# alexoz12v2/cuda-optix-pathtracing

Measured on AMD Instinct MI355X. Metric: Msamples/s (paths x spp / s), higher is better.
Workload: dtype f32

## Files before the change

### cuda-optix-pathtracing_amd/binding.py

```python
import ctypes as C
import subprocess
from pathlib import Path

import numpy as np

_HERE = Path(__file__).resolve().parent
_CSRC = _HERE / "csrc"
_LIB = None

DMT_ACCEL_BRUTE_FORCE = 0
DMT_ACCEL_BVH = 1
BVH_BUILD_HOST = 0
BVH_BUILD_DEVICE = 1
BVH_BUILT_BY_HOST = 0
BVH_BUILT_BY_DEVICE = 1
BVH_BUILT_BY_HOST_AFTER_DEVICE = 2
BVH_UPDATE_REBUILD = 0
BVH_UPDATE_REFIT = 1
BVH_UPDATE_AUTO = 2
BVH_UPDATED_NONE = 0
BVH_UPDATED_REFIT = 1
BVH_UPDATED_REBUILD = 2
BVH_UPDATED_REBUILD_AFTER_REFIT = 3


class DmtError(RuntimeError):
    pass


def library_path():
    import os
    alt = os.environ.get("DMT_HIP_LIB")
    return Path(alt) if alt else _CSRC / "libdmt_hip.so"


def build_library(force=False):
    args = ["make", "-C", str(_CSRC)]
    if force:
        args.append("-B")
    subprocess.check_call(args)
    return library_path()


def load_library():
    global _LIB
    if _LIB is None:
        so = library_path()
        if not so.exists():
            raise DmtError(f"{so} is missing: run `python -c 'import __graft_entry__ as g; g.build()'` "
                           "(the HIP path has no fallback)")
        lib = C.CDLL(str(so))
        lib.dmt_last_error.restype = C.c_char_p
        lib.dmt_last_error.argtypes = [C.c_void_p]
        _LIB = lib
    return _LIB


EXPORTED_SYMBOLS = [
    "dmt_ctx_create", "dmt_ctx_destroy", "dmt_last_error", "dmt_upload_triangles", "dmt_upload_bsdfs",
    "dmt_upload_lights", "dmt_set_camera", "dmt_set_limits", "dmt_set_accel", "dmt_set_light_sampling", "dmt_light_tree_pmfs", "dmt_light_tree_ref_select", "dmt_set_bvh_strategy", "dmt_set_partition", "dmt_set_chunk", "dmt_render_profile",
    "dmt_upload_area_lights", "dmt_upload_textures", "dmt_upload_envmap", "dmt_clear_envmap", "dmt_envmap_tables", "dmt_test_envmap",
    "dmt_set_stream", "dmt_film_clear", "dmt_film_bind", "dmt_film_device_ptrs", "dmt_download_film",
    "dmt_render", "dmt_render_adaptive", "dmt_render_stats", "dmt_sync", "dmt_sched_diag", "dmt_kernel_time", "dmt_kernel_info", "dmt_bvh_validate", "dmt_brute_cull_plan", "dmt_brute_cull_box_plan", "dmt_test_triangle_intersect",
    "dmt_test_sampler", "dmt_test_camera_rays", "dmt_test_bsdf", "dmt_test_bsdf_ng", "dmt_test_material", "dmt_test_light", "dmt_test_half",
    "dmt_test_trace_samples", "dmt_test_trace_log", "dmt_test_closest_hit",
    "dmt_set_texture_filter", "dmt_texture_mip_chain", "dmt_texture_footprint", "dmt_test_texture_filter",
    "dmt_render_aovs", "dmt_upload_aovs", "dmt_download_aovs", "dmt_denoise_defaults", "dmt_denoise",
    "dmt_set_accel_build", "dmt_accel_build_info", "dmt_accel_download", "dmt_lbvh_reference", "dmt_bvh_check",
    "dmt_update_vertices", "dmt_update_vertices_device", "dmt_set_accel_update", "dmt_accel_update_info", "dmt_bvh_refit_reference",
    "dmt_download_aov_surface", "dmt_upload_aov_surface", "dmt_camera_project", "dmt_test_camera_project", "dmt_temporal_defaults",
    "dmt_denoise_temporal", "dmt_temporal_reset", "dmt_temporal_info", "dmt_temporal_download",
    "dmt_set_sampler_table", "dmt_sampler_table_plan", "dmt_test_sampler_table",
]

SAMPLER_TABLE_OFF = 0
SAMPLER_TABLE_AUTO = 1
SAMPLER_TABLE_FORCE = 2


class SamplerTablePlanRecord(C.Structure):
    _fields_ = [("use", C.c_uint32), ("period_width", C.c_uint32), ("period_height", C.c_uint32), ("entry_bytes", C.c_uint32),
                ("slices", C.c_uint32), ("reserved", C.c_uint32), ("slice_bytes", C.c_uint64)]


def sampler_table_plan(width, height, owned_pixels, spp, chunk_spp, budget_bytes=0, mode=SAMPLER_TABLE_AUTO):
    lib = load_library()
    rec = SamplerTablePlanRecord()
    args = [int(width), int(height), C.c_uint64(int(owned_pixels)), C.c_uint32(int(spp)), C.c_uint32(int(chunk_spp)),
            C.c_uint64(int(budget_bytes)), int(mode)]
    rc = lib.dmt_sampler_table_plan(*args, C.byref(rec), None, C.c_uint32(0))
    if rc != 0:
        raise DmtError(f"dmt_sampler_table_plan failed ({rc})")
    lens = (C.c_uint32 * max(int(rec.slices), 1))()
    rc = lib.dmt_sampler_table_plan(*args, C.byref(rec), lens, C.c_uint32(int(rec.slices)))
    if rc != 0:
        raise DmtError(f"dmt_sampler_table_plan failed ({rc})")
    out = {name: int(getattr(rec, name)) for name, _ in SamplerTablePlanRecord._fields_ if name != "reserved"}
    out["use"] = bool(rec.use)
    out["slice_spp"] = [int(x) for x in lens[:int(rec.slices)]]
    return out


class DenoiseParams(C.Structure):
    _fields_ = [("iterations", C.c_int32), ("sigma_normal", C.c_float), ("sigma_position", C.c_float),
                ("sigma_albedo", C.c_float), ("sigma_luminance", C.c_float)]


def denoise_defaults():
    lib = load_library()
    lib.dmt_denoise_defaults.restype = DenoiseParams
    p = lib.dmt_denoise_defaults()
    return {name: getattr(p, name) for name, _ in DenoiseParams._fields_}



class TemporalParams(C.Structure):
    _fields_ = [("alpha", C.c_float), ("normal_threshold", C.c_float), ("plane_threshold", C.c_float)]


class TemporalRecord(C.Structure):
    _fields_ = [("frames", C.c_uint32), ("reprojected", C.c_uint32), ("reset", C.c_uint32), ("temporal_ms", C.c_float),
                ("history_bytes", C.c_uint64)]


def temporal_defaults():
    lib = load_library()
    lib.dmt_temporal_defaults.restype = TemporalParams
    p = lib.dmt_temporal_defaults()
    return {name: getattr(p, name) for name, _ in TemporalParams._fields_}


def camera_project(camera44, points):
    lib = load_library()
    cam = np.ascontiguousarray(camera44, np.uint8).reshape(44)
    p = np.ascontiguousarray(points, np.float32).reshape(-1, 3)
    xy, depth = np.zeros((p.shape[0], 2), np.float32), np.zeros(p.shape[0], np.float32)
    rc = lib.dmt_camera_project(cam.ctypes.data_as(C.c_void_p), int(p.shape[0]), p.ctypes.data_as(C.c_void_p),
                                xy.ctypes.data_as(C.c_void_p), depth.ctypes.data_as(C.c_void_p))
    if rc != 0:
        raise DmtError(f"dmt_camera_project failed ({rc})")
    return xy, depth


TEXFILTER_LEVEL0 = 0
TEXFILTER_REFERENCE = 1


def mip_level_count(width, height):
# ... 565 lines not shown
        prep = np.zeros((n, 12), np.float32)
        samp = np.zeros((n, 10), np.float32)
        ev = np.zeros((n, 4), np.float32)
        self._check(self._lib.dmt_test_bsdf_ng(self._ctx, _p(b), n, _p(ns), _p(ng), _p(wo), _p(u2), _p(uc), _p(wi_eval),
                                               _p(prep), _p(samp), _p(ev)), "dmt_test_bsdf_ng")
        return prep, samp, ev

    def test_material(self, tri, bu, bv, ng):
        tri, bu, bv, ng = _i32(tri), _f32(bu, (-1,)), _f32(bv, (-1,)), _f32(ng, (-1, 3))
        n = tri.shape[0]
        assert bu.shape[0] == n and bv.shape[0] == n and ng.shape[0] == n
        rec, rec2 = np.zeros((n, 32), np.uint8), np.zeros((n, 32), np.uint8)
        ns = np.zeros((n, 3), np.float32)
        mix = np.zeros(n, np.float32)
        self._check(self._lib.dmt_test_material(self._ctx, n, _p(tri), _p(bu), _p(bv), _p(ng), _p(rec), _p(ns), _p(rec2),
                                                _p(mix)), "dmt_test_material")
        return rec, ns, rec2, mix

    def test_light(self, light32, pos, nrm, u2, had_t):
        l = np.ascontiguousarray(light32, np.uint8).reshape(32)
        pos, nrm, u2 = _f32(pos, (-1, 3)), _f32(nrm, (-1, 3)), _f32(u2, (-1, 2))
        ht = _i32(had_t)
        n = pos.shape[0]
        out = np.zeros((n, 14), np.float32)
        self._check(self._lib.dmt_test_light(self._ctx, _p(l), n, _p(pos), _p(nrm), _p(u2), _p(ht), _p(out)),
                    "dmt_test_light")
        return out

    def test_half(self, floats=None, halves=None):
        h_out = f_out = None
        n = 0
        if floats is not None:
            floats = _f32(floats, (-1,))
            n = floats.shape[0]
            h_out = np.zeros(n, np.uint16)
        if halves is not None:
            halves = np.ascontiguousarray(halves, np.uint16).reshape(-1)
            n = halves.shape[0]
            f_out = np.zeros(n, np.float32)
        if floats is not None and halves is not None:
            assert floats.shape[0] == halves.shape[0]
        self._check(self._lib.dmt_test_half(self._ctx, n, _p(floats), _p(h_out), _p(halves), _p(f_out)),
                    "dmt_test_half")
        return h_out, f_out

    def test_trace_samples(self, pxs, pys, ss):
        pxs, pys, ss = _i32(pxs), _i32(pys), _i32(ss)
        n = pxs.shape[0]
        out = np.zeros((n, 3), np.float32)
        self._check(self._lib.dmt_test_trace_samples(self._ctx, n, _p(pxs), _p(pys), _p(ss), _p(out)),
                    "dmt_test_trace_samples")
        return out

    def test_texture_filter(self, tri, bu, bv, tex, depth=0):
        tri, tex = _i32(tri), _i32(tex)
        bu, bv = _f32(bu), _f32(bv)
        n = tri.shape[0]
        tex = np.ascontiguousarray(np.broadcast_to(tex, (n,)), np.int32)
        depth = np.ascontiguousarray(np.broadcast_to(_i32(depth), (n,)), np.int32)
        assert bu.shape[0] == n and bv.shape[0] == n
        rgb = np.zeros((n, 3), np.float32)
        branch = np.zeros(n, np.int32)
        lod = np.zeros(n, np.float32)
        self._check(self._lib.dmt_test_texture_filter(self._ctx, n, _p(tri), _p(bu), _p(bv), _p(tex), _p(depth), _p(rgb),
                                                      _p(branch), _p(lod)), "dmt_test_texture_filter")
        return rgb, branch, lod

    def test_trace_log(self, px, py, s, cap=64):
        rec = np.zeros((cap, 12), np.float32)
        n = C.c_int()
        L = np.zeros(3, np.float32)
        self._check(self._lib.dmt_test_trace_log(self._ctx, int(px), int(py), int(s), _p(rec), int(cap), C.byref(n),
                                                 _p(L)), "dmt_test_trace_log")
        return rec[:n.value], L

    def test_closest_hit(self, o, d):
        o, d = _f32(o, (-1, 3)), _f32(d, (-1, 3))
        n = o.shape[0]
        idx = np.zeros(n, np.int32)
        t = np.zeros(n, np.float32)
        self._check(self._lib.dmt_test_closest_hit(self._ctx, n, _p(o), _p(d), _p(idx), _p(t)),
                    "dmt_test_closest_hit")
        return idx, t
```

### cuda-optix-pathtracing_amd/csrc/dmt_hip.hip

```cpp
#include <hip/hip_runtime.h>

#include <algorithm>
#include <chrono>
#include <cmath>
#include <cstddef>
#include <cstdio>
#include <cstdlib>
#include <cstring>
#include <limits>
#include <memory>
#include <new>
#include <string>
#include <vector>

#include "../../include/dmt_hip.h"
#include "pt_device.hpp"
#include "bvh_device.hpp"
#include "bvh_gpu_build.hpp"
#include "devbuf.hpp"
#include "envmap.hpp"
#include "light_tree.hpp"
#include "light_tree_ref.hpp"

using namespace dmt;
// ... 835 lines not shown
        }
        set_shadow_ray(st, offset_ray_origin(hit.pos, hit.error, hit.normal, ls.direction), ls.direction);
        st.smax = ls.distance;
        st.hasShadow = true;
      }
    }
  }

  sect_mark(7);
  f2 const u2 = st.rng.get2D();
  float const uc = st.rng.get1D();
  BsdfSample bs = sample_bsdf(b, wo, ns, hit.normal, u2, uc);
  if constexpr (F & kFeatBlend) {
    if (blend) {
      BsdfSample sC = sample_bsdf(b2, wo, ns, hit.normal, u2, uc);
      sC.f = bs.f * (1.f - mix) + sC.f * mix;
      sC.pdf = blend_pdf(bs.pdf, sC.pdf);
      sC.eta = 1.f;
      bs = sC;
    }
  }
  sect_mark(8);
  if (!bs.valid()) return true;
  st.lastT = bs.refract;
  if constexpr (F & (kFeatEnv | kFeatArea)) st.lastPdf = bs.pdf, st.lastSpecular = bs.delta;
  set_ray(st, offset_ray_origin(hit.pos, hit.error, hit.normal, bs.wi), bs.wi);
  st.beta = st.beta * (bs.f * fabsf(dot(bs.wi, hit.normal)) / bs.pdf);
  float const rrBeta = max3(st.beta * bs.eta);
  if (rrBeta < 1 && st.depth > 1) {
    float const q = fmaxf(0.f, 1.f - rrBeta);
    if (st.rng.get1D() < q) return true;
    st.beta = st.beta / (1 - q);
  }
  ++st.depth;
  sect_mark(9);
  return false;
}

DMT_DEV TriS load_tri(TriIsect const DMT_CONST_AS* tris, uint32_t i) {
  TriS T;
  T.p0x = tris[i].p0x, T.p0y = tris[i].p0y, T.p0z = tris[i].p0z;
  T.e0x = tris[i].e0x, T.e0y = tris[i].e0y, T.e0z = tris[i].e0z;
  T.e1x = tris[i].e1x, T.e1y = tris[i].e1y, T.e1z = tris[i].e1z;
  return T;
}

struct BruteHit {
  float bt, bu, bv;
  int tri;
  bool occluded;
};
#define DMT_TRI_DECL(P) float P##0, P##1, P##2, P##3, P##4, P##5, P##6, P##7, P##8
#define DMT_TRI_LOAD(P, idx)                                                                          \
  P##0 = tris[idx].p0x, P##1 = tris[idx].p0y, P##2 = tris[idx].p0z, P##3 = tris[idx].e0x, P##4 = tris[idx].e0y, \
  P##5 = tris[idx].e0z, P##6 = tris[idx].e1x, P##7 = tris[idx].e1y, P##8 = tris[idx].e1z
#define DMT_TRI_TEST(P, idx)                                                                                   \
  do {                                                                                                         \
    MTPair m;                                                                                                  \
    mt_core9<v2f>(P##0, P##1, P##2, P##3, P##4, P##5, P##6, P##7, P##8, st.rp.ox, st.rp.oy, st.rp.oz, st.rp.dx, \
                  st.rp.dy, st.rp.dz, m.det, m.t, m.u, m.v);                                                   \
    bool const v1 = mt_valid(m.det.x, m.t.x, m.u.x, m.v.x);                                                    \
    bool const v2 = mt_valid(m.det.y, m.t.y, m.u.y, m.v.y);                                                    \
    if (doC && v1 && m.t.x < h.bt) {                  \
      h.bt = m.t.x;                                                                                            \
      h.tri = int(idx);                                                                                        \
      h.bu = m.u.x;                                                                                            \
      h.bv = m.v.x;                                                                                            \
    }                                                                                                          \
    if (doS && v2 && m.t.y < st.smax) h.occluded = true;                                         \
  } while (0)

__shared__ float s_cullTri[9 * kCullMaxTris];
__shared__ CullRec s_cullRec[kCullMaxClusters];
__shared__ unsigned long long s_cullKey[kLdsThreads];
__shared__ unsigned long long s_cullOcc[kLdsThreads / 64];
__shared__ uint8_t s_cullOwner[kLdsThreads / 64][kCullGroup][128];
constexpr float kCullTSlack = 1.0f + 1.0f / 256;
constexpr float kCullRel = 1.0f / 16384;
constexpr float kCullTLo = 1e-4f * (1.0f - 1.0f / 256);

#ifndef DMT_CULL_COUNTS
#define DMT_CULL_COUNTS 0
#endif
#if DMT_CULL_COUNTS
__device__ unsigned long long g_cullCount[16];
#endif

DMT_DEV void cull_stage(KArgs k) {
  k = kargs(k);
  if (k->cull.clusterCount == 0) return;
  float const* const t9 = k->cull.tri9;
  for (uint32_t i = threadIdx.x; i < 9 * kCullMaxTris; i += blockDim.x) s_cullTri[i] = t9[i];
  CullCluster const* const cl = k->cull.clusters;
  for (uint32_t i = threadIdx.x; i < kCullMaxClusters; i += blockDim.x)
    s_cullRec[i] = CullRec{cl[i].first, cl[i].count | cl[i].slot << 16, cl[i].magic};
  __syncthreads();
}

DMT_DEV float slab_rcp(float d) { return rcp_(copysignf(fmaxf(fabsf(d), 0x1p-126f), d)); }

DMT_DEV void brute_clusters(KArgs k, PathState const& st, bool doC, bool doS, BruteHit& h) {
  k = kargs(k);
  uint32_t const nc = k->cull.clusterCount;
  auto const* const cls = to_const_as(k->cull.clusters);
  if (h.tri >= 0) h.tri = int(k->cull.alwaysIdx[h.tri]);
  uint32_t const lane = threadIdx.x & 63u, w = threadIdx.x >> 6;
  unsigned long long const act = __ballot(1);
  uint32_t const nAct = uint32_t(__popcll(act));
  uint32_t const rank = __builtin_amdgcn_mbcnt_hi(uint32_t(act >> 32), __builtin_amdgcn_mbcnt_lo(uint32_t(act), 0u));
  s_cullKey[threadIdx.x] = ~0ull;
  s_cullOcc[w] = 0;
  float tmaxC = h.bt * kCullTSlack;
  float const tmaxS = st.smax * kCullTSlack;
  v2f const ix = {slab_rcp(st.rp.dx.x), slab_rcp(st.rp.dx.y)};
  v2f const iy = {slab_rcp(st.rp.dy.x), slab_rcp(st.rp.dy.y)};
  v2f const iz = {slab_rcp(st.rp.dz.x), slab_rcp(st.rp.dz.y)};
#if DMT_CULL_COUNTS
  unsigned long long cnt[16] = {};
  cnt[0] = 1, cnt[1] = __popcll(__ballot(doC)), cnt[2] = __popcll(__ballot(doS));
#endif
  for (uint32_t c0 = 0; c0 < nc; c0 += kCullGroup) {
    uint32_t pre[kCullGroup + 1];
    pre[0] = 0;
#pragma unroll
    for (uint32_t q = 0; q < kCullGroup; ++q) {
      uint32_t tasks = 0;
      if (c0 + q < nc) {
        auto const& r = cls[c0 + q];
        CullCluster cl;
        for (int i = 0; i < 6; ++i) cl.b[i] = r.b[i];
        cl.box = r.box, cl.count = r.count;
        bool hitC, hitS;
        if (cl.box) {
          v2f const x0 = (cl.b[0] - st.rp.ox) * ix, x1 = (cl.b[3] - st.rp.ox) * ix;
          v2f const y0 = (cl.b[1] - st.rp.oy) * iy, y1 = (cl.b[4] - st.rp.oy) * iy;
          v2f const z0 = (cl.b[2] - st.rp.oz) * iz, z1 = (cl.b[5] - st.rp.oz) * iz;
          float const nC = fmaxf(fmaxf(fminf(x0.x, x1.x), fminf(y0.x, y1.x)), fmaxf(fminf(z0.x, z1.x), kCullTLo));
          float const fC = fminf(fminf(fmaxf(x0.x, x1.x), fmaxf(y0.x, y1.x)), fminf(fmaxf(z0.x, z1.x), tmaxC));
          float const nS = fmaxf(fmaxf(fminf(x0.y, x1.y), fminf(y0.y, y1.y)), fmaxf(fminf(z0.y, z1.y), kCullTLo));
          float const fS = fminf(fminf(fmaxf(x0.y, x1.y), fmaxf(y0.y, y1.y)), fminf(fmaxf(z0.y, z1.y), tmaxS));
          hitC = doC && nC <= fC * kCullTSlack, hitS = doS && nS <= fS * kCullTSlack;
        } else {
          v2f const wx = cl.b[0] - st.rp.ox, wy = cl.b[1] - st.rp.oy, wz = cl.b[2] - st.rp.oz;
          v2f const dd = st.rp.dx * st.rp.dx + st.rp.dy * st.rp.dy + st.rp.dz * st.rp.dz;
          v2f const ww = wx * wx + wy * wy + wz * wz;
          v2f tc = (wx * st.rp.dx + wy * st.rp.dy + wz * st.rp.dz) * rcp_(dd);
          tc.x = fminf(fmaxf(tc.x, 0.f), tmaxC);
          tc.y = fminf(fmaxf(tc.y, 0.f), tmaxS);
          v2f const ex = wx - tc * st.rp.dx, ey = wy - tc * st.rp.dy, ez = wz - tc * st.rp.dz;
          v2f const ee = ex * ex + ey * ey + ez * ez;
          v2f const lim = cl.b[3] + kCullRel * (ww + tc * tc * dd);
          hitC = doC && ee.x <= lim.x, hitS = doS && ee.y <= lim.y;
        }
        unsigned long long const mC = __ballot(hitC), mS = __ballot(hitS);
        uint32_t const nC = uint32_t(__popcll(mC)), nS = uint32_t(__popcll(mS));
        if (hitC) s_cullOwner[w][q][__builtin_amdgcn_mbcnt_hi(uint32_t(mC >> 32), __builtin_amdgcn_mbcnt_lo(uint32_t(mC), 0u))] = uint8_t(lane);
        if (hitS)
          s_cullOwner[w][q][nC + __builtin_amdgcn_mbcnt_hi(uint32_t(mS >> 32), __builtin_amdgcn_mbcnt_lo(uint32_t(mS), 0u))] =
              uint8_t(lane | 64u);
        tasks = (nC + nS) * cl.count;
#if DMT_CULL_COUNTS
        if (cl.box) cnt[5] += nC, cnt[7] += nS, cnt[9] += tasks;
        else cnt[4] += nC, cnt[6] += nS, cnt[8] += tasks;
#endif
      }
      pre[q + 1] = pre[q] + tasks;
    }
    uint32_t const total = pre[kCullGroup];
#if DMT_CULL_COUNTS
    cnt[3] += (total + nAct - 1) / nAct;
#endif
    asm volatile("" ::: "memory");
    for (uint32_t base = 0; base < total; base += nAct) {
      uint32_t const g = min(base + rank, total - 1u);
      uint32_t q = 0, first = 0;
#pragma unroll
      for (uint32_t p = 1; p < kCullGroup; ++p)
        if (g >= pre[p]) q = p, first = pre[p];
      CullRec const rec = s_cullRec[c0 + q];
      uint32_t const count = rec.countSlot & 0xFFFFu, slot0 = rec.countSlot >> 16;
      uint32_t const local = g - first;
      uint32_t const e = __umulhi(local, rec.magic);
      uint32_t const j = local - e * count;
      uint32_t const own = s_cullOwner[w][q][e];
      bool const shadow = own >= 64u;
      int const src = int(own & 63u) << 2;
      auto pull = [&](v2f v) {
        float const a = __int_as_float(__builtin_amdgcn_ds_bpermute(src, __float_as_int(v.x)));
        float const b = __int_as_float(__builtin_amdgcn_ds_bpermute(src, __float_as_int(v.y)));
        return shadow ? b : a;
      };
      float const ox = pull(st.rp.ox), oy = pull(st.rp.oy), oz = pull(st.rp.oz);
      float const dx = pull(st.rp.dx), dy = pull(st.rp.dy), dz = pull(st.rp.dz);
      float const smax = __int_as_float(__builtin_amdgcn_ds_bpermute(src, __float_as_int(st.smax)));
      float const* const T = s_cullTri + slot0 + j;
      float det, t, u, v;
      mt_core9<float>(T[0 * kCullMaxTris], T[1 * kCullMaxTris], T[2 * kCullMaxTris], T[3 * kCullMaxTris], T[4 * kCullMaxTris],
                      T[5 * kCullMaxTris], T[6 * kCullMaxTris], T[7 * kCullMaxTris], T[8 * kCullMaxTris], ox, oy, oz, dx, dy, dz,
                      det, t, u, v);
      if (base + rank < total && mt_valid(det, t, u, v)) {
        if (shadow) {
          if (t < smax) atomicOr(&s_cullOcc[w], 1ull << (own & 63u));
        } else if (t < kInf) {
          atomicMin(&s_cullKey[w * 64u + own],
                    (static_cast<unsigned long long>(__float_as_uint(t)) << 32) | ((rec.first + j) << kCullSlotBits) | (slot0 + j));
        }
      }
    }
    asm volatile("" ::: "memory");
    if (c0 + kCullGroup < nc) {
      unsigned long long const kc = s_cullKey[threadIdx.x];
      if (kc != ~0ull) tmaxC = fminf(tmaxC, __uint_as_float(uint32_t(kc >> 32)) * kCullTSlack);
    }
  }
#if DMT_CULL_COUNTS
  if (rank == 0)
    for (int i = 0; i < 10; ++i) atomicAdd(&g_cullCount[i], cnt[i]);
#endif
  if (doC) {
    unsigned long long const kc = s_cullKey[threadIdx.x];
    if (kc < ((static_cast<unsigned long long>(__float_as_uint(h.bt)) << 32) | (uint32_t(h.tri) << kCullSlotBits))) {
      float const* const T = s_cullTri + (uint32_t(kc) & ((1u << kCullSlotBits) - 1u));
      float det, t, u, v;
      mt_core9<float>(T[0 * kCullMaxTris], T[1 * kCullMaxTris], T[2 * kCullMaxTris], T[3 * kCullMaxTris], T[4 * kCullMaxTris],
                      T[5 * kCullMaxTris], T[6 * kCullMaxTris], T[7 * kCullMaxTris], T[8 * kCullMaxTris], st.rp.ox.x, st.rp.oy.x,
                      st.rp.oz.x, st.rp.dx.x, st.rp.dy.x, st.rp.dz.x, det, t, u, v);
      h.bt = __uint_as_float(uint32_t(kc >> 32)), h.tri = int(uint32_t(kc) >> kCullSlotBits), h.bu = u, h.bv = v;
    }
  }
  if (doS && ((s_cullOcc[w] >> lane) & 1ull)) h.occluded = true;
}

template <bool CULL>
DMT_DEV void trace_pair_brute(KArgs k, PathState const& st, bool doC, bool doS, int& bestTri, float& bu,
                              float& bv, bool& occluded) {
  BruteHit h{kInf, 0.f, 0.f, -1, false};
  k = kargs(k);
  auto const* tris = to_const_as(CULL ? k->cull.always : k->scene.tris);
  uint32_t const n = CULL ? k->cull.alwaysCount : k->scene.triCount;
  uint32_t const last = n ? n - 1 : 0;
  DMT_TRI_DECL(a);
  DMT_TRI_DECL(b);
  DMT_TRI_LOAD(a, 0);
  for (uint32_t i = 0; i < n;) {
    uint32_t const ib = i + 1 < last ? i + 1 : last;
    DMT_TRI_LOAD(b, ib);
    __builtin_amdgcn_sched_barrier(0);
    DMT_TRI_TEST(a, i);
    if (++i >= n) break;
    uint32_t const ia = i + 1 < last ? i + 1 : last;
    DMT_TRI_LOAD(a, ia);
    __builtin_amdgcn_sched_barrier(0);
    DMT_TRI_TEST(b, i);
    ++i;
  }
  if constexpr (CULL) {
    if (kargs(k)->cull.clusterCount != 0) brute_clusters(k, st, doC, doS, h);
  }
  bestTri = h.tri, bu = h.bu, bv = h.bv, occluded = h.occluded;
}

struct LaneStats {
  uint32_t samples = 0, closest = 0, shadow = 0, bounces = 0;
  TraversalCounters tc;
  uint32_t itNode = 0, itLeaf = 0, itShade = 0, itOuter = 0, itPrep = 0, lanesLeaf = 0, lanesShade = 0, lanesPrep = 0;
};
template <bool STATS = false>
DMT_DEV void trace_pair_bvh(KArgs k, PathState const& st, bool doC, bool doS, uint32_t gtid, int& bestTri,
                            float& bu, float& bv, bool& occluded, LaneStats* ls = nullptr) {
  BvhView const bvh = load_bvh(k);
  float bt;
  if constexpr (STATS) ls->closest += doC ? 1u : 0u, ls->shadow += doS ? 1u : 0u;
  bvh_closest<STATS>(bvh, doC, mk3(st.rp.ox.x, st.rp.oy.x, st.rp.oz.x), mk3(st.rp.dx.x, st.rp.dy.x, st.rp.dz.x),
                     gtid, bestTri, bt, bu, bv, STATS ? &ls->tc : nullptr);
  occluded = bvh_any<STATS>(bvh, doS, mk3(st.rp.ox.y, st.rp.oy.y, st.rp.oz.y),
                            mk3(st.rp.dx.y, st.rp.dy.y, st.rp.dz.y), st.smax, gtid, STATS ? &ls->tc : nullptr);
}

template <uint32_t F, class Sink>
DMT_DEV void lane_finish(KArgs k, PathState& st, bool doC, bool doS, int bestTri, float bu, float bv, bool occluded,
                         Sink&& sink);

template <uint32_t F, class Sink>
DMT_DEV void lane_step(KArgs k, uint32_t gtid, PathState& st, Sink&& sink, LaneStats* ls = nullptr) {
  bool const doC = st.active;
  bool const doS = st.hasShadow;
  int bestTri;
  float bu, bv;
  bool occluded;
  if constexpr (F & kFeatBvh)
    trace_pair_bvh<(F & kFeatStats) != 0>(k, st, doC, doS, gtid, bestTri, bu, bv, occluded, ls);
  else
    trace_pair_brute(k, st, doC, doS, bestTri, bu, bv, occluded);
  sect_mark(2);
  if constexpr (F & kFeatStats) ls->bounces += (doC && bestTri >= 0 && st.depth < kargs(k)->maxDepth) ? 1u : 0u;
  lane_finish<F & ~kFeatStats>(k, st, doC, doS, bestTri, bu, bv, occluded, sink);
}

template <uint32_t F, class Sink>
DMT_DEV void lane_finish(KArgs k, PathState& st, bool doC, bool doS, int bestTri, float bu, float bv, bool occluded,
// ... 3204 lines not shown
```

### cuda-optix-pathtracing_amd/csrc/probes.hpp

```cpp
#pragma once

#include "probe_stage.hpp"

namespace {

template <uint32_t F>
__global__ void k_test_trace(RenderParams P, int n, int32_t const* pxs, int32_t const* pys, int32_t const* ss, float* L3) {
  KArgs const k = kargs_base();
  if constexpr (!(F & kFeatBvh)) cull_stage(k);
  int const i = int(blockIdx.x * blockDim.x + threadIdx.x);
  PathState st{};
  if (i < n) {
    ColdArgs const c = load_cold_args(k);
    path_begin(st, c.cam, c.sp, pxs[i], pys[i], halton_pixel_base(c.sp, pxs[i], pys[i]), uint32_t(ss[i]));
  }
  auto store = [&](f3 L, uint32_t) { L3[3 * i] = L.x, L3[3 * i + 1] = L.y, L3[3 * i + 2] = L.z; };
  uint32_t const gtid = blockIdx.x * blockDim.x + threadIdx.x;
  while (__any(st.active || st.hasShadow)) lane_step<F>(k, gtid, st, store);
}

__global__ void k_test_texfilter(RenderParams P, int n, int32_t const* tri, float const* bu, float const* bv, int32_t const* tex,
                                 int32_t const* depth, float* rgb3, int32_t* branch, float* lod) {
#pragma clang fp contract(off)
  KArgs const k = kargs_base();
// ... 149 lines not shown
__global__ void k_test_bsdf(Rec32 rec, int n, float const* ns3, float const* wo3, float const* u2, float const* uc, float const* wi3,
                            float* prep12, float* samp10, float* eval4) {
  test_bsdf_body<false>(rec, n, ns3, nullptr, wo3, u2, uc, wi3, prep12, samp10, eval4);
}

__global__ void k_test_bsdf_ng(Rec32 rec, int n, float const* ns3, float const* ng3, float const* wo3, float const* u2,
                               float const* uc, float const* wi3, float* prep12, float* samp10, float* eval4) {
  test_bsdf_body<true>(rec, n, ns3, ng3, wo3, u2, uc, wi3, prep12, samp10, eval4);
}

__global__ void k_test_material(RenderParams P, int n, int32_t const* tri, float const* bu, float const* bv, float const* ng3,
                                uint32_t* rec8, float* ns3, uint32_t* rec2_8, float* mixOut) {
  KArgs const k = kargs_base();
  int const i = int(blockIdx.x * blockDim.x + threadIdx.x);
  if (i >= n) return;
  SceneView const sc = load_scene(k);
  uint32_t const matId = sc.post[tri[i]].matId;
  f3 const ng = mk3(ng3[3 * i], ng3[3 * i + 1], ng3[3 * i + 2]);
  Rec32 rec = sc.bsdfs[matId], rec2{};
  float mix = 0.f;
  bool const blend = hi16(rec.w[1]) == BS_GGX_BLEND && matId + 1u < sc.bsdfCount;
  if (blend) {
    mix = blend_metallic<false>(k, rec, matId, tri[i], bu[i], bv[i]);
    rec.w[1] = (rec.w[1] & 0x0000FFFFu) | (uint32_t(BS_GGX_DIEL) << 16);
    rec2 = sc.bsdfs[matId + 1u];
  }
  f3 ns = ng;
  if (kargs(k)->matTex != nullptr) {
    ns = apply_material_textures<false>(k, rec, matId, tri[i], bu[i], bv[i], ng);
    if (blend) (void)apply_material_textures<false>(k, rec2, matId + 1u, tri[i], bu[i], bv[i], ng);
  }
  if (blend) rec.w[1] = (rec.w[1] & 0x0000FFFFu) | (uint32_t(BS_GGX_BLEND) << 16);
  for (int w = 0; w < 8; ++w) rec8[8 * size_t(i) + w] = rec.w[w], rec2_8[8 * size_t(i) + w] = rec2.w[w];
  ns3[3 * i] = ns.x, ns3[3 * i + 1] = ns.y, ns3[3 * i + 2] = ns.z;
  mixOut[i] = mix;
}

__global__ void k_test_light(Rec32 rec, int n, float const* pos3, float const* nrm3, float const* u2,
                             int32_t const* hadT, float* out14) {
  int const i = int(blockIdx.x * blockDim.x + threadIdx.x);
  if (i >= n) return;
  LightSample const s = sample_light(rec, mk3(pos3[3 * i], pos3[3 * i + 1], pos3[3 * i + 2]),
                                     mk2(u2[2 * i], u2[2 * i + 1]), hadT[i] != 0,
                                     mk3(nrm3[3 * i], nrm3[3 * i + 1], nrm3[3 * i + 2]));
  f3 const Le = eval_light(rec, s);
  float* o = out14 + 14 * size_t(i);
  o[0] = s.pLight.x, o[1] = s.pLight.y, o[2] = s.pLight.z;
  o[3] = s.direction.x, o[4] = s.direction.y, o[5] = s.direction.z;
  o[6] = s.pdf, o[7] = float(s.delta), o[8] = s.distance, o[9] = s.factor;
  o[10] = Le.x, o[11] = Le.y, o[12] = Le.z, o[13] = s.valid() ? 1.f : 0.f;
}

__global__ void k_test_half(int n, float const* fin, uint16_t* hout, uint16_t const* hin, float* fout) {
  int const i = int(blockIdx.x * blockDim.x + threadIdx.x);
  if (i >= n) return;
  if (fin && hout) hout[i] = uint16_t(f2h(fin[i]));
  if (hin && fout) fout[i] = h2f(hin[i]);
}

__global__ void k_test_closest(RenderParams P, bool useBvh, int n, float const* o3, float const* d3, int32_t* tri,
                               float* tOut) {
  KArgs const k = kargs_base();
  if (!useBvh) cull_stage(k);
  int const i = int(blockIdx.x * blockDim.x + threadIdx.x);
  bool const alive = i < n;
  PathState st{};
  if (alive)
    set_ray(st, mk3(o3[3 * i], o3[3 * i + 1], o3[3 * i + 2]), mk3(d3[3 * i], d3[3 * i + 1], d3[3 * i + 2]));
  st.active = alive;
  int best;
  float bu, bv, bt = kInf;
  bool occluded;
  if (useBvh)
    trace_pair_bvh(k, st, alive, false, blockIdx.x * blockDim.x + threadIdx.x, best, bu, bv, occluded);
  else
    trace_pair_brute(k, st, alive, false, best, bu, bv, occluded);
  if (alive && best >= 0) {
    TriS const T = load_tri(to_const_as(load_scene(k).tris), uint32_t(best));
    bt = mt_pair(T, st.rp).t.x;
  }
  if (alive) tri[i] = best, tOut[i] = bt;
}

__global__ void k_test_project(ProjXf c, int n, float const* p3, float* xy2, float* depth) {
  int const i = int(blockIdx.x * blockDim.x + threadIdx.x);
  if (i >= n) return;
  Proj const o = project_point(c, p3[3 * i], p3[3 * i + 1], p3[3 * i + 2]);
  xy2[2 * i] = o.fx, xy2[2 * i + 1] = o.fy, depth[i] = o.depth;
}

typedef void (*TestTraceFn)(RenderParams, int, int32_t const*, int32_t const*, int32_t const*, float*);
#define DMT_TEST_TRACE_ROW(suffix, mask, waves, body) {mask, k_test_trace<mask>},
KernelRow<TestTraceFn> const kTestTraceKernels[] = {DMT_MEGAKERNELS(DMT_TEST_TRACE_ROW)};

int probeError(dmt_ctx* ctx, Probe const& p) {
  ctx->err = std::string(p.call) + ": " + hipGetErrorName(p.err) + " - " + hipGetErrorString(p.err);
  return DMT_ERR_HIP;
}

int finishProbe(dmt_ctx* ctx, Probe& p) {
  if (int const rc = finishTest(ctx)) return rc;
  return p.fetch() == hipSuccess ? DMT_OK : probeError(ctx, p);
}

int sceneReady(dmt_ctx* ctx, char const* who, bool wholeScene) {
  if (wholeScene && !(ctx->haveTris && ctx->haveBsdfs && ctx->haveLights && ctx->haveCamera))
    return fail(ctx, DMT_ERR_STATE, (std::string(who) + ": scene/camera not set").c_str());
  if (ctx->triCount > 0 && ctx->maxMatId >= ctx->bsdfCount)
    return fail(ctx, DMT_ERR_INVALID, (std::string(who) + ": material index outside the BSDF array").c_str());
  return DMT_OK;
}

int probeBsdf(dmt_ctx* ctx, void const* bsdf32, int n, float const* ns3, float const* ng3, float const* wo3, float const* u2,
              float const* uc, float const* wi_eval3, float* prepared12, float* sample10, float* eval4) {
  if (n == 0) return DMT_OK;
  Probe p(ctx->device, size_t(n));
  ProbeIn<float> dns(p, ns3, 3), dng(p, ng3, 3), dwo(p, wo3, 3), du2(p, u2, 2), duc(p, uc, 1), dwi(p, wi_eval3, 3);
  ProbeOut<float> dp(p, prepared12, 12), ds(p, sample10, 10), de(p, eval4, 4);
  if (p.err != hipSuccess) return probeError(ctx, p);
  Rec32 rec;
  memcpy(&rec, bsdf32, 32);
  if (ng3)
    hipLaunchKernelGGL(k_test_bsdf_ng, dim3(p.blocks(64)), dim3(64), 0, ctx->stream, rec, n, dns.get(), dng.get(), dwo.get(), du2.get(),
                       duc.get(), dwi.get(), dp.get(), ds.get(), de.get());
  else
    hipLaunchKernelGGL(k_test_bsdf, dim3(p.blocks(64)), dim3(64), 0, ctx->stream, rec, n, dns.get(), dwo.get(), du2.get(), duc.get(),
                       dwi.get(), dp.get(), ds.get(), de.get());
  return finishProbe(ctx, p);
}

}

extern "C" {

int dmt_test_envmap(dmt_ctx* ctx, int n, const float* u2, const float* wi_in3, float* wi3, float* pdf, float* uv2, float* Le3,
                    int32_t* ok, float* Le_dir3, float* pdf_dir) {
  if (!ctx || n <= 0 || !u2 || !wi_in3 || !wi3 || !pdf || !uv2 || !Le3 || !ok || !Le_dir3 || !pdf_dir) return DMT_ERR_INVALID;
  if (ctx->env.w <= 0) return fail(ctx, DMT_ERR_STATE, "dmt_test_envmap: no env map uploaded");
  Probe p(ctx->device, size_t(n));
  ProbeIn<float> du(p, u2, 2), dwin(p, wi_in3, 3);
  ProbeOut<float> dwi(p, wi3, 3), dpdf(p, pdf, 1), duv(p, uv2, 2), dLe(p, Le3, 3), dLd(p, Le_dir3, 3), dpd(p, pdf_dir, 1);
  ProbeOut<int32_t> dok(p, ok, 1);
  if (p.err != hipSuccess) return probeError(ctx, p);
  hipLaunchKernelGGL(k_test_envmap, dim3(p.blocks(64)), dim3(64), 0, ctx->stream, ctx->env, n, du.get(), dwin.get(), dwi.get(),
                     dpdf.get(), duv.get(), dLe.get(), dok.get(), dLd.get(), dpd.get());
  return finishProbe(ctx, p);
}

int dmt_test_sampler_table(dmt_ctx* ctx, int width, int height, uint32_t s0, uint32_t n, float* out_vals, float* out_jitter) {
  if (!ctx || width <= 0 || height <= 0 || !out_vals || !out_jitter) return DMT_ERR_INVALID;
  uint32_t const pw = uint32_t(width < 128 ? width : 128), ph = uint32_t(height < 128 ? height : 128);
  SamplerParams const sp = computeSamplerParams(width, height);
  if (uint64_t(n) * pw * ph > 0x7FFFFFFFull || (uint64_t(s0) + n + 1) * uint64_t(sp.scale0) * uint64_t(sp.scale1) > 0x7FFFFFFFull)
    return fail(ctx, DMT_ERR_INVALID, "dmt_test_sampler_table: too many entries, or the sample index overflows the 32-bit Halton index");
  if (n == 0) return DMT_OK;
  Probe p(ctx->device, size_t(n) * pw * ph);
  ProbeOut<float4> dv(p, out_vals, 2);
  ProbeOut<float2> dj(p, out_jitter, 1);
  if (p.err != hipSuccess) return probeError(ctx, p);
  hipLaunchKernelGGL(k_sampler_table, dim3(p.blocks(256)), dim3(256), 0, ctx->stream, sp, s0, n, pw, ph, dv.get(), dj.get());
  return finishProbe(ctx, p);
}

int dmt_test_triangle_intersect(dmt_ctx* ctx, const float* xs, const float* ys, const float* zs, size_t count, const float* o3,
                                const float* d3, int32_t* hit, float* t, float* pos3, float* nrm3, float* err3) {
  if (!ctx || !xs || !ys || !zs || !o3 || !d3 || !hit) return DMT_ERR_INVALID;
// ... 104 lines not shown
  if (n == 0) return DMT_OK;
  Probe p(ctx->device, size_t(n));
  ProbeIn<float> dfi(p, f_in, 1);
  ProbeOut<uint16_t> dho(p, h_out, f_in && h_out ? 1 : 0);
  ProbeIn<uint16_t> dhi(p, h_in, 1);
  ProbeOut<float> dfo(p, f_out, h_in && f_out ? 1 : 0);
  if (p.err != hipSuccess) return probeError(ctx, p);
  hipLaunchKernelGGL(k_test_half, dim3(p.blocks(256)), dim3(256), 0, ctx->stream, n, dfi.get(), dho.get(), dhi.get(), dfo.get());
  return finishProbe(ctx, p);
}

int dmt_test_trace_samples(dmt_ctx* ctx, int n, const int32_t* pxs, const int32_t* pys, const int32_t* ss, float* L3) {
  if (!ctx || n < 0 || !pxs || !pys || !ss || !L3) return DMT_ERR_INVALID;
  if (int const rc = sceneReady(ctx, "dmt_test_trace_samples", true)) return rc;
  if (n == 0) return DMT_OK;
  Probe p(ctx->device, size_t(n));
  ProbeIn<int32_t> dpx(p, pxs, 1), dpy(p, pys, 1), dss(p, ss, 1);
  ProbeOut<float> dL(p, L3, 3);
  if (p.err != hipSuccess) return probeError(ctx, p);
  uint32_t F = 0;
  if (int const rc = resolveFeatures(ctx, &F)) return rc;
  TestTraceFn const kernel = kernelOf(kTestTraceKernels, F);
  if (!kernel) return noKernel(ctx, "dmt_test_trace_samples", F);
  if (F & kFeatBvh) {
    if (!ctx->haveBvh) return fail(ctx, DMT_ERR_STATE, "dmt_test_trace_samples: BVH not built");
    HIP_TRY(ctx, reserveOverflow(ctx, p.threads(64)));
  }
  hipLaunchKernelGGL(kernel, dim3(p.blocks(64)), dim3(64), 0, ctx->stream, baseParams(ctx, p.threads(64)), n, dpx.get(), dpy.get(),
                     dss.get(), dL.get());
  return finishProbe(ctx, p);
}

int dmt_test_texture_filter(dmt_ctx* ctx, int n, const int32_t* tri, const float* bu, const float* bv, const int32_t* tex,
                            const int32_t* depth, float* rgb3, int32_t* branch, float* lod) {
  if (!ctx || n < 0 || !tri || !bu || !bv || !tex || !depth || !rgb3 || !branch || !lod) return DMT_ERR_INVALID;
  if (!(ctx->haveTris && ctx->haveCamera) || ctx->texCount == 0 || ctx->triUvCount != ctx->triCount)
    return fail(ctx, DMT_ERR_STATE, "dmt_test_texture_filter: triangles, camera and textures (with one UV triple per triangle) first");
  for (int i = 0; i < n; ++i)
    if (tri[i] < 0 || size_t(tri[i]) >= ctx->triCount || tex[i] < 0 || uint32_t(tex[i]) >= ctx->texCount)
      return fail(ctx, DMT_ERR_INVALID, "dmt_test_texture_filter: triangle or texture index out of range");
  if (n == 0) return DMT_OK;
  Probe p(ctx->device, size_t(n));
  ProbeIn<int32_t> dTri(p, tri, 1), dTex(p, tex, 1), dDepth(p, depth, 1);
  ProbeIn<float> dBu(p, bu, 1), dBv(p, bv, 1);
  ProbeOut<float> dRgb(p, rgb3, 3), dLod(p, lod, 1);
  ProbeOut<int32_t> dBranch(p, branch, 1);
  if (p.err != hipSuccess) return probeError(ctx, p);
  hipLaunchKernelGGL(k_test_texfilter, dim3(p.blocks(64)), dim3(64), 0, ctx->stream, baseParams(ctx, p.threads(64)), n, dTri.get(),
                     dBu.get(), dBv.get(), dTex.get(), dDepth.get(), dRgb.get(), dBranch.get(), dLod.get());
  return finishProbe(ctx, p);
}

int dmt_test_trace_log(dmt_ctx* ctx, int px, int py, int s, float* rec12, int cap, int* n_out, float* L3) {
  if (!ctx || !rec12 || cap <= 0 || !n_out || !L3) return DMT_ERR_INVALID;
  if (int const rc = sceneReady(ctx, "dmt_test_trace_log", true)) return rc;
  Probe p(ctx->device, 1);
  ProbeOut<float> dr(p, rec12, 12 * size_t(cap)), dL(p, L3, 3);
  ProbeOut<int> dn(p, n_out, 1);
  if (p.err != hipSuccess) return probeError(ctx, p);
  hipLaunchKernelGGL(k_test_trace_log, dim3(p.blocks(64)), dim3(64), 0, ctx->stream, baseParams(ctx, p.threads(64)), px, py, s, dr.get(),
                     cap, dn.get(), dL.get());
  return finishProbe(ctx, p);
}

int dmt_test_closest_hit(dmt_ctx* ctx, int nrays, const float* o3, const float* d3, int32_t* tri_index, float* t) {
  if (!ctx || nrays < 0 || !o3 || !d3 || !tri_index || !t) return DMT_ERR_INVALID;
  if (!ctx->haveTris) return fail(ctx, DMT_ERR_STATE, "dmt_test_closest_hit: upload triangles first");
  if (nrays == 0) return DMT_OK;
  Probe p(ctx->device, size_t(nrays));
  ProbeIn<float> dO(p, o3, 3), dD(p, d3, 3);
  ProbeOut<int32_t> di(p, tri_index, 1);
  ProbeOut<float> dt(p, t, 1);
  if (p.err != hipSuccess) return probeError(ctx, p);
  bool const useBvh = ctx->accel == DMT_ACCEL_BVH;
  if (useBvh) {
    if (!ctx->haveBvh) return fail(ctx, DMT_ERR_STATE, "dmt_test_closest_hit: BVH not built");
    HIP_TRY(ctx, reserveOverflow(ctx, p.threads(64)));
  }
  hipLaunchKernelGGL(k_test_closest, dim3(p.blocks(64)), dim3(64), 0, ctx->stream, baseParams(ctx, p.threads(64)), useBvh, nrays,
                     dO.get(), dD.get(), di.get(), dt.get());
  return finishProbe(ctx, p);
}

}
```

### include/dmt_hip.h

```cpp
#ifndef DMT_HIP_H
#define DMT_HIP_H

#include <stddef.h>
#include <stdint.h>

#ifdef __cplusplus
extern "C" {
#endif

typedef struct dmt_ctx dmt_ctx;

typedef struct dmt_camera {
  float dir[3];
  float pos[3];
  int32_t width;
  int32_t height;
  int32_t spp;
  float focal_length;
  float sensor_size;
} dmt_camera;

enum {
  DMT_OK = 0,
  DMT_ERR_INVALID = 1,
// ... 128 lines not shown
  DMT_BVH_UPDATED_REBUILD_AFTER_REFIT = 3,
};
typedef struct dmt_accel_update_record {
  int32_t action;
  uint32_t updates_since_build;
  double update_ms;
  double sah_cost;
  double sah_cost_at_build;
  uint64_t temp_bytes;
} dmt_accel_update_record;
int dmt_accel_update_info(dmt_ctx* ctx, dmt_accel_update_record* out);
int dmt_bvh_refit_reference(const void* nodes64, size_t node_count, const uint32_t* pair_orig2, size_t pair_count,
                            const float* xs, const float* ys, const float* zs, size_t count, void* nodes64_out);

int dmt_brute_cull_plan(const float* xs, const float* ys, const float* zs, const uint32_t* mat_id, size_t count,
                        int enable, uint32_t* cluster_count, uint32_t* cluster_first_count, float* cluster_sphere);

int dmt_brute_cull_box_plan(const float* xs, const float* ys, const float* zs, const uint32_t* mat_id, size_t count,
                            int enable, uint32_t* cluster_count, uint32_t* cluster_first_count, float* cluster_box);

int dmt_render_aovs(dmt_ctx* ctx, uint32_t aov_spp);
int dmt_upload_aovs(dmt_ctx* ctx, const float* albedo4, const float* normal4, const float* position4, int width, int height);
int dmt_download_aovs(dmt_ctx* ctx, float* albedo4, float* normal4, float* position4);
typedef struct dmt_denoise_params {
  int32_t iterations;
  float sigma_normal;
  float sigma_position;
  float sigma_albedo;
  float sigma_luminance;
} dmt_denoise_params;
dmt_denoise_params dmt_denoise_defaults(void);
int dmt_denoise(dmt_ctx* ctx, const dmt_denoise_params* params, const float* mean4, const float* m24, float* out4, float* kernel_ms);

int dmt_download_aov_surface(dmt_ctx* ctx, float* surface4);
int dmt_upload_aov_surface(dmt_ctx* ctx, const float* surface4, int width, int height);
int dmt_camera_project(const dmt_camera* cam, int n, const float* p3, float* xy2, float* depth);
typedef struct dmt_temporal_params {
  float alpha;
  float normal_threshold;
  float plane_threshold;
} dmt_temporal_params;
dmt_temporal_params dmt_temporal_defaults(void);
int dmt_denoise_temporal(dmt_ctx* ctx, const dmt_denoise_params* params, const dmt_temporal_params* tparams, const float* mean4,
                         const float* m24, float* out4, float* kernel_ms);
int dmt_temporal_reset(dmt_ctx* ctx);
typedef struct dmt_temporal_record {
  uint32_t frames;
  uint32_t reprojected;
  uint32_t reset;
  float temporal_ms;
  uint64_t history_bytes;
} dmt_temporal_record;
int dmt_temporal_info(dmt_ctx* ctx, dmt_temporal_record* out);
int dmt_temporal_download(dmt_ctx* ctx, float* color_var4, float* length1);

int dmt_test_triangle_intersect(dmt_ctx* ctx, const float* xs, const float* ys, const float* zs,
                                size_t count, const float* o3, const float* d3, int32_t* hit,
                                float* t, float* pos3, float* nrm3, float* err3);
int dmt_test_sampler(dmt_ctx* ctx, int width, int height, int n, const int32_t* pxs,
                     const int32_t* pys, const int32_t* ss, int ndims, int32_t* halton_index,
                     float* pixel2d, float* dims);
int dmt_test_sampler_table(dmt_ctx* ctx, int width, int height, uint32_t s0, uint32_t n, float* out_vals, float* out_jitter);
int dmt_test_camera_rays(dmt_ctx* ctx, int n, const int32_t* pxs, const int32_t* pys,
                         const int32_t* ss, float* o3, float* d3);
int dmt_test_camera_project(dmt_ctx* ctx, int n, const float* p3, float* xy2, float* depth);
int dmt_test_bsdf(dmt_ctx* ctx, const void* bsdf32, int n, const float* ns3, const float* wo3,
                  const float* u2, const float* uc, const float* wi_eval3, float* prepared12,
                  float* sample10, float* eval4);
int dmt_test_bsdf_ng(dmt_ctx* ctx, const void* bsdf32, int n, const float* ns3, const float* ng3, const float* wo3,
                     const float* u2, const float* uc, const float* wi_eval3, float* prepared12, float* sample10,
                     float* eval4);
int dmt_test_material(dmt_ctx* ctx, int n, const int32_t* tri, const float* bu, const float* bv, const float* ng3, void* rec32,
                      float* ns3, void* rec2_32, float* mix);
int dmt_test_light(dmt_ctx* ctx, const void* light32, int n, const float* pos3, const float* nrm3,
                   const float* u2, const int32_t* had_transmission, float* out14);
int dmt_test_half(dmt_ctx* ctx, int n, const float* f_in, uint16_t* h_out, const uint16_t* h_in,
                  float* f_out);
int dmt_test_trace_samples(dmt_ctx* ctx, int n, const int32_t* pxs, const int32_t* pys,
                           const int32_t* ss, float* L3);
int dmt_test_trace_log(dmt_ctx* ctx, int px, int py, int s, float* rec12, int cap, int* n_out,
                       float* L3);
int dmt_test_closest_hit(dmt_ctx* ctx, int nrays, const float* o3, const float* d3,
                         int32_t* tri_index, float* t);

#ifdef __cplusplus
}
#endif
#endif
```

Baseline: 5785.

## Test two triangles per task in brute-force cluster culling

The culled brute-force intersection loop now hands each lane a pair of adjacent triangles per task, so the task count per cluster is halved. The ray origin, direction and smax are fetched by bpermute once and reused for both triangles, and the per-cluster magic divisor is recomputed for units instead of single triangles. This cuts the per-task overhead of decoding, shuffles and LDS atomics, but odd counts leave a masked slot and per-task register pressure rises. A new test entry point validates the paired trace against the reference.

Result: no change. 5837, median of 6 (+0.9%).

```diff
diff --git a/cuda-optix-pathtracing_amd/binding.py b/cuda-optix-pathtracing_amd/binding.py
--- a/cuda-optix-pathtracing_amd/binding.py
+++ b/cuda-optix-pathtracing_amd/binding.py
@@ -63,7 +63,7 @@
     "dmt_set_stream", "dmt_film_clear", "dmt_film_bind", "dmt_film_device_ptrs", "dmt_download_film",
     "dmt_render", "dmt_render_adaptive", "dmt_render_stats", "dmt_sync", "dmt_sched_diag", "dmt_kernel_time", "dmt_kernel_info", "dmt_bvh_validate", "dmt_brute_cull_plan", "dmt_brute_cull_box_plan", "dmt_test_triangle_intersect",
     "dmt_test_sampler", "dmt_test_camera_rays", "dmt_test_bsdf", "dmt_test_bsdf_ng", "dmt_test_material", "dmt_test_light", "dmt_test_half",
-    "dmt_test_trace_samples", "dmt_test_trace_log", "dmt_test_closest_hit",
+    "dmt_test_trace_samples", "dmt_test_trace_log", "dmt_test_closest_hit", "dmt_test_trace_pair",
     "dmt_set_texture_filter", "dmt_texture_mip_chain", "dmt_texture_footprint", "dmt_test_texture_filter",
     "dmt_render_aovs", "dmt_upload_aovs", "dmt_download_aovs", "dmt_denoise_defaults", "dmt_denoise",
     "dmt_set_accel_build", "dmt_accel_build_info", "dmt_accel_download", "dmt_lbvh_reference", "dmt_bvh_check",
@@ -795,3 +795,15 @@
         self._check(self._lib.dmt_test_closest_hit(self._ctx, n, _p(o), _p(d), _p(idx), _p(t)),
                     "dmt_test_closest_hit")
         return idx, t
+
+    def test_trace_pair(self, o, d, so, sd, smax):
+        o, d, so, sd = (_f32(a, (-1, 3)) for a in (o, d, so, sd))
+        smax = _f32(smax)
+        n = o.shape[0]
+        assert d.shape[0] == n and so.shape[0] == n and sd.shape[0] == n and smax.shape[0] == n
+        idx = np.zeros(n, np.int32)
+        tuv = np.zeros((n, 3), np.float32)
+        occ = np.zeros(n, np.int32)
+        self._check(self._lib.dmt_test_trace_pair(self._ctx, n, _p(o), _p(d), _p(so), _p(sd), _p(smax), _p(idx), _p(tuv),
+                                                  _p(occ)), "dmt_test_trace_pair")
+        return idx, tuv[:, 0].copy(), tuv[:, 1].copy(), tuv[:, 2].copy(), occ.astype(bool)
diff --git a/cuda-optix-pathtracing_amd/csrc/dmt_hip.hip b/cuda-optix-pathtracing_amd/csrc/dmt_hip.hip
--- a/cuda-optix-pathtracing_amd/csrc/dmt_hip.hip
+++ b/cuda-optix-pathtracing_amd/csrc/dmt_hip.hip
@@ -941,6 +941,13 @@
 #ifndef DMT_CULL_COUNTS
 #define DMT_CULL_COUNTS 0
 #endif
+#ifndef DMT_CULL_PAIRS
+#define DMT_CULL_PAIRS 1
+#endif
+constexpr uint32_t kCullUnitShift = 20;
+static_assert(128u * ((kCullMaxTris + 1u) / 2u) * ((kCullMaxTris + 1u) / 2u) < (1u << kCullUnitShift) &&
+              128u * ((kCullMaxTris + 1u) / 2u) < (1u << (32 - kCullUnitShift)), "unit decode of brute_clusters");
+DMT_HD constexpr uint32_t cull_units(uint32_t count) { return (count + 1u) >> 1; }
 #if DMT_CULL_COUNTS
 __device__ unsigned long long g_cullCount[16];
 #endif
@@ -951,8 +958,15 @@
   float const* const t9 = k->cull.tri9;
   for (uint32_t i = threadIdx.x; i < 9 * kCullMaxTris; i += blockDim.x) s_cullTri[i] = t9[i];
   CullCluster const* const cl = k->cull.clusters;
-  for (uint32_t i = threadIdx.x; i < kCullMaxClusters; i += blockDim.x)
-    s_cullRec[i] = CullRec{cl[i].first, cl[i].count | cl[i].slot << 16, cl[i].magic};
+  for (uint32_t i = threadIdx.x; i < kCullMaxClusters; i += blockDim.x) {
+#if DMT_CULL_PAIRS
+    uint32_t const units = max(cull_units(cl[i].count), 1u);
+    uint32_t const magic = ((1u << kCullUnitShift) + units - 1u) / units;
+#else
+    uint32_t const magic = cl[i].magic;
+#endif
+    s_cullRec[i] = CullRec{cl[i].first, cl[i].count | cl[i].slot << 16, magic};
+  }
   __syncthreads();
 }
 
@@ -1017,10 +1031,11 @@
         if (hitS)
           s_cullOwner[w][q][nC + __builtin_amdgcn_mbcnt_hi(uint32_t(mS >> 32), __builtin_amdgcn_mbcnt_lo(uint32_t(mS), 0u))] =
               uint8_t(lane | 64u);
-        tasks = (nC + nS) * cl.count;
+        tasks = (nC + nS) * (DMT_CULL_PAIRS ? cull_units(cl.count) : cl.count);
 #if DMT_CULL_COUNTS
-        if (cl.box) cnt[5] += nC, cnt[7] += nS, cnt[9] += tasks;
-        else cnt[4] += nC, cnt[6] += nS, cnt[8] += tasks;
+        if (cl.box) cnt[5] += nC, cnt[7] += nS, cnt[9] += (nC + nS) * cl.count;
+        else cnt[4] += nC, cnt[6] += nS, cnt[8] += (nC + nS) * cl.count;
+        cnt[10] += tasks;
 #endif
       }
       pre[q + 1] = pre[q] + tasks;
@@ -1030,6 +1045,53 @@
     cnt[3] += (total + nAct - 1) / nAct;
 #endif
     asm volatile("" ::: "memory");
+#if DMT_CULL_PAIRS
+    for (uint32_t base = 0; base < total; base += nAct) {
+      uint32_t const g = min(base + rank, total - 1u);
+      uint32_t q = 0, first = 0;
+#pragma unroll
+      for (uint32_t p = 1; p < kCullGroup; ++p)
+        if (g >= pre[p]) q = p, first = pre[p];
+      CullRec const rec = s_cullRec[c0 + q];
+      uint32_t const count = rec.countSlot & 0xFFFFu, slot0 = rec.countSlot >> 16;
+      uint32_t const local = g - first;
+      uint32_t const e = __umul24(local, rec.magic) >> kCullUnitShift;
+      uint32_t const p2 = 2u * (local - __umul24(e, cull_units(count)));
+      bool const full = p2 + 1u < count;
+      uint32_t const j = full ? p2 : p2 - 1u;
+      uint32_t const own = s_cullOwner[w][q][e];
+      bool const shadow = own >= 64u;
+      int const src = int(own & 63u) << 2;
+      auto bperm = [&](float v) { return __int_as_float(__builtin_amdgcn_ds_bpermute(src, __float_as_int(v))); };
+      auto pull = [&](v2f v) {
+        float const a = bperm(v.x), b = bperm(v.y);
+        return shadow ? b : a;
+      };
+      float const ox = pull(st.rp.ox), oy = pull(st.rp.oy), oz = pull(st.rp.oz);
+      float const dx = pull(st.rp.dx), dy = pull(st.rp.dy), dz = pull(st.rp.dz);
+      float const smax = bperm(st.smax);
+      float const* const T = s_cullTri + slot0 + j;
+      constexpr uint32_t S = kCullMaxTris;
+      bool const live = base + rank < total;
+      float detA, tA, uA, vA, detB, tB, uB, vB;
+      mt_core9<float>(T[0 * S], T[1 * S], T[2 * S], T[3 * S], T[4 * S], T[5 * S], T[6 * S], T[7 * S], T[8 * S], ox, oy, oz, dx,
+                      dy, dz, detA, tA, uA, vA);
+      bool const okA = live && full && mt_valid(detA, tA, uA, vA);
+      mt_core9<float>(T[0 * S + 1], T[1 * S + 1], T[2 * S + 1], T[3 * S + 1], T[4 * S + 1], T[5 * S + 1], T[6 * S + 1],
+                      T[7 * S + 1], T[8 * S + 1], ox, oy, oz, dx, dy, dz, detB, tB, uB, vB);
+      bool const okB = live && mt_valid(detB, tB, uB, vB);
+      if (shadow) {
+        if ((okA && tA < smax) || (okB && tB < smax)) atomicOr(&s_cullOcc[w], 1ull << (own & 63u));
+      } else {
+        uint32_t const lo = ((rec.first + j) << kCullSlotBits) | (slot0 + j);
+        unsigned long long const kA = okA && tA < kInf ? (static_cast<unsigned long long>(__float_as_uint(tA)) << 32) | lo : ~0ull;
+        unsigned long long const kB =
+            okB && tB < kInf ? (static_cast<unsigned long long>(__float_as_uint(tB)) << 32) | (lo + (1u << kCullSlotBits) + 1u) : ~0ull;
+        unsigned long long const kk = kA < kB ? kA : kB;
+        if (kk != ~0ull) atomicMin(&s_cullKey[w * 64u + own], kk);
+      }
+    }
+#else
     for (uint32_t base = 0; base < total; base += nAct) {
       uint32_t const g = min(base + rank, total - 1u);
       uint32_t q = 0, first = 0;
@@ -1066,6 +1128,7 @@
         }
       }
     }
+#endif
     asm volatile("" ::: "memory");
     if (c0 + kCullGroup < nc) {
       unsigned long long const kc = s_cullKey[threadIdx.x];
@@ -1074,7 +1137,7 @@
   }
 #if DMT_CULL_COUNTS
   if (rank == 0)
-    for (int i = 0; i < 10; ++i) atomicAdd(&g_cullCount[i], cnt[i]);
+    for (int i = 0; i < 11; ++i) atomicAdd(&g_cullCount[i], cnt[i]);
 #endif
   if (doC) {
     unsigned long long const kc = s_cullKey[threadIdx.x];
diff --git a/cuda-optix-pathtracing_amd/csrc/probes.hpp b/cuda-optix-pathtracing_amd/csrc/probes.hpp
--- a/cuda-optix-pathtracing_amd/csrc/probes.hpp
+++ b/cuda-optix-pathtracing_amd/csrc/probes.hpp
@@ -255,6 +255,34 @@
   if (alive) tri[i] = best, tOut[i] = bt;
 }
 
+__global__ void __launch_bounds__(kLdsThreads) k_test_trace_pair(RenderParams P, int n, float const* o3, float const* d3,
+                                                                 float const* so3, float const* sd3, float const* smax,
+                                                                 int32_t* tri, float* tuv3, int32_t* occ) {
+  KArgs const k = kargs_base();
+  cull_stage(k);
+  int const i = int(blockIdx.x * blockDim.x + threadIdx.x);
+  bool const alive = i < n;
+  PathState st{};
+  if (alive) {
+    set_ray(st, mk3(o3[3 * i], o3[3 * i + 1], o3[3 * i + 2]), mk3(d3[3 * i], d3[3 * i + 1], d3[3 * i + 2]));
+    set_shadow_ray(st, mk3(so3[3 * i], so3[3 * i + 1], so3[3 * i + 2]), mk3(sd3[3 * i], sd3[3 * i + 1], sd3[3 * i + 2]));
+    st.smax = smax[i];
+  }
+  st.active = alive;
+  int best;
+  float bu, bv, bt = kInf;
+  bool occluded;
+  trace_pair_brute(k, st, alive, alive, best, bu, bv, occluded);
+  if (!alive) return;
+  if (best >= 0) {
+    TriS const T = load_tri(to_const_as(load_scene(k).tris), uint32_t(best));
+    bt = mt_pair(T, st.rp).t.x;
+  } else {
+    bu = bv = 0.f;
+  }
+  tri[i] = best, tuv3[3 * i] = bt, tuv3[3 * i + 1] = bu, tuv3[3 * i + 2] = bv, occ[i] = occluded ? 1 : 0;
+}
+
 __global__ void k_test_project(ProjXf c, int n, float const* p3, float* xy2, float* depth) {
   int const i = int(blockIdx.x * blockDim.x + threadIdx.x);
   if (i >= n) return;
@@ -525,4 +553,21 @@
   return finishProbe(ctx, p);
 }
 
-}
+int dmt_test_trace_pair(dmt_ctx* ctx, int nrays, const float* o3, const float* d3, const float* so3, const float* sd3,
+                        const float* smax, int32_t* tri_index, float* tuv3, int32_t* occluded) {
+  if (!ctx || nrays < 0 || !o3 || !d3 || !so3 || !sd3 || !smax || !tri_index || !tuv3 || !occluded) return DMT_ERR_INVALID;
+  if (!ctx->haveTris) return fail(ctx, DMT_ERR_STATE, "dmt_test_trace_pair: upload triangles first");
+  if (ctx->accel == DMT_ACCEL_BVH) return fail(ctx, DMT_ERR_STATE, "dmt_test_trace_pair: the brute-force pass only");
+  if (nrays == 0) return DMT_OK;
+  Probe p(ctx->device, size_t(nrays));
+  ProbeIn<float> dO(p, o3, 3), dD(p, d3, 3), dSo(p, so3, 3), dSd(p, sd3, 3), dSmax(p, smax, 1);
+  ProbeOut<int32_t> di(p, tri_index, 1), dOcc(p, occluded, 1);
+  ProbeOut<float> dt(p, tuv3, 3);
+  if (p.err != hipSuccess) return probeError(ctx, p);
+  hipLaunchKernelGGL(k_test_trace_pair, dim3(p.blocks(kLdsThreads)), dim3(kLdsThreads), 0, ctx->stream,
+                     baseParams(ctx, p.threads(kLdsThreads)), nrays, dO.get(), dD.get(), dSo.get(), dSd.get(), dSmax.get(), di.get(),
+                     dt.get(), dOcc.get());
+  return finishProbe(ctx, p);
+}
+
+}
diff --git a/include/dmt_hip.h b/include/dmt_hip.h
--- a/include/dmt_hip.h
+++ b/include/dmt_hip.h
@@ -234,6 +234,9 @@
                        float* L3);
 int dmt_test_closest_hit(dmt_ctx* ctx, int nrays, const float* o3, const float* d3,
                          int32_t* tri_index, float* t);
+int dmt_test_trace_pair(dmt_ctx* ctx, int nrays, const float* o3, const float* d3, const float* so3,
+                        const float* sd3, const float* smax, int32_t* tri_index, float* tuv3,
+                        int32_t* occluded);
 
 #ifdef __cplusplus
 }
```
